# imalexlee/simple-vk-renderer

Hardware: AMD Instinct MI355X
Metric: shaded fragments/s (higher is better)
Workload: dtype f32

## Files before the change

simple-vk-renderer_amd/csrc/k_bin.hip:

```cpp
#include <hip/hip_ext.h>

#include <algorithm>

#include "svr_bin.h"
#include "svr_clip.h"
#include "svr_launch.h"

namespace svr {

__device__ __forceinline__ EdgeSet load_edges(const TriRec* rec) {
  EdgeSet e;
  const double2* p = reinterpret_cast<const double2*>(rec);
  double2 a = p[2], b = p[3], c = p[4], d = p[5];
  e.A0 = a.x; e.A1 = a.y; e.A2 = b.x; e.B0 = b.y; e.B1 = c.x; e.B2 = c.y; e.C0 = d.x; e.C1 = d.y;
  e.C2 = rec->C[2];
  return e;
}

struct RecBox {
  int minx, miny, maxx, maxy;
  uint32_t flags;
  bool valid;
};
__device__ __forceinline__ RecBox load_box(const TriRec* rec) {
  uint4 h = *reinterpret_cast<const uint4*>(rec);
  RecBox b;
  b.minx = (int)(int16_t)(h.x & 0xffffu);
  b.miny = (int)(int16_t)(h.x >> 16);
  b.maxx = (int)(int16_t)(h.y & 0xffffu);
  b.maxy = (int)(int16_t)(h.y >> 16);
  b.flags = h.w;
  b.valid = b.minx <= b.maxx;
  return b;
}

__device__ __forceinline__ void bin_one(const FrameParams& P, uint32_t r, int minx, int miny, int maxx, int maxy, uint32_t binbase,
                                        const EdgeSet& e, uint32_t n_setup) {
  const uint32_t lane = threadIdx.x & 63u;
  const unsigned long long below = (1ull << lane) - 1ull;
// ... 89 lines not shown
      bool made = false;
      uint32_t rec = 0, transparent = 0;
      if (worker && i + 1 < np) {
        const DrawDesc& d = P.draws[draw];
        ScreenV s0 = to_screen(poly[0].clip, hw, hh), s1 = to_screen(poly[i].clip, hw, hh), s2 = to_screen(poly[i + 1].clip, hw, hh);
        if (s0.ok && s1.ok && s2.ok && poly[0].clip[3] > 0.0f && poly[i].clip[3] > 0.0f && poly[i + 1].clip[3] > 0.0f) {
          rec = P.n_tris + first + used;
          uint4* dst = reinterpret_cast<uint4*>(P.recs + rec);
          if (setup_triangle(P, &poly[0], &poly[i], &poly[i + 1], s0, s1, s2, make_key(seq, d.flags, P.tex[d.tex], true), d.flags, P.tex[d.tex],
                             *reinterpret_cast<uint4(*)[16]>(dst), &L.geom[lane])) {
            made = true;
            used++;
            if (IDS) *reinterpret_cast<uint2*>(dst + REC_ID_PIECE) = make_uint2(d.pad, prim);
            transparent = MV ? bin_base<true>(P, d.flags) : ((d.flags & F_TRANSPARENT) ? 1u : 0u);
            if (P.instrument) atomicAdd(&P.counters->binned, 1ull);
          }
        }
      }
      __builtin_amdgcn_fence(__ATOMIC_RELEASE, "wavefront");
      __builtin_amdgcn_wave_barrier();
      for (unsigned long long todo = __ballot(made); todo; todo &= todo - 1ull) {
        const int l = __ffsll((long long)todo) - 1;
        const TriGeom& gm = L.geom[l];
        EdgeSet e;
        e.A0 = gm.A[0]; e.A1 = gm.A[1]; e.A2 = gm.A[2]; e.B0 = gm.B[0]; e.B1 = gm.B[1]; e.B2 = gm.B[2];
        e.C0 = gm.C[0]; e.C1 = gm.C[1]; e.C2 = gm.C[2];
        bin_one(P, (uint32_t)__shfl((int)rec, l), gm.minx, gm.miny, gm.maxx, gm.maxy, MV ? (uint32_t)__shfl((int)transparent, l) : (__shfl((int)transparent, l) ? P.n_tiles : 0u), e, n_setup);
      }
      __builtin_amdgcn_wave_barrier();
    }
    if (worker && np >= 3) {
      for (uint32_t k = used; k < want; k++) store_invalid(P.recs + P.n_tris + first + k);
      uint4 link;
      link.x = 1u;
      link.y = 0u;
      link.z = P.n_tris + first;
      link.w = used;
      *reinterpret_cast<uint4*>(P.recs + seq) = link;
    }
  }
}

template <bool IDS, bool MV>
__device__ __forceinline__ void count_main(const FrameParams& P, uint32_t big_blocks, uint32_t clip_blocks) {
  __shared__ ClipLds s_clip;
  if (P.counters->overflow) return;
  if (blockIdx.x < big_blocks) {
    bin_big<MV>(P, (blockIdx.x * blockDim.x + threadIdx.x) >> 6, (big_blocks * blockDim.x) >> 6);
    return;
// ... 183 lines not shown
```

simple-vk-renderer_amd/csrc/k_geometry.hip:

```cpp
#include <algorithm>

#include "svr_bin.h"
#include "svr_clip.h"
#include "svr_launch.h"

namespace svr {

__device__ __forceinline__ bool chunk_can_be_seen(const FrameParams& P, const float* mvp, const float lo[3], const float hi[3], uint32_t lane) {
  const float px = (lane & 4u) ? hi[0] : lo[0], py = (lane & 2u) ? hi[1] : lo[1], pz = (lane & 1u) ? hi[2] : lo[2];
  float c[4];
  matvec4(mvp, px, py, pz, 1.0f, c);
  const float inv_hw = 2.0f / (float)P.W, inv_hh = 2.0f / (float)P.H;
  const float x_lo = ((float)P.sx - 1.0f) * inv_hw - 1.0f, x_hi = ((float)(P.sx + P.sw) + 1.0f) * inv_hw - 1.0f;
  const float y_lo = ((float)P.sy - 1.0f) * inv_hh - 1.0f, y_hi = ((float)(P.sy + P.sh) + 1.0f) * inv_hh - 1.0f;
  const unsigned long long corners = 0xffull;
  const bool out_near = c[2] > c[3], out_far = c[2] < 0.0f;
  const bool out_l = c[0] < x_lo * c[3], out_r = c[0] > x_hi * c[3];
  const bool out_t = c[1] < y_lo * c[3], out_b = c[1] > y_hi * c[3];
  const bool gone = (__ballot(out_near) & corners) == corners || (__ballot(out_far) & corners) == corners ||
                    (__ballot(out_l) & corners) == corners || (__ballot(out_r) & corners) == corners ||
                    (__ballot(out_t) & corners) == corners || (__ballot(out_b) & corners) == corners;
  if (gone) return false;
  if (P.rstride > 1u) {
    const bool front = (__ballot(c[3] > 0.0f) & corners) == corners;
// ... 191 lines not shown
      piece[REC_ID_PIECE].x = d.pad;
      piece[REC_ID_PIECE].y = tri;
    }
    if (ok && P.instrument) atomicAdd(&P.counters->binned, 1ull);
    if (to_clip) {
      uint32_t slot = atomicAdd(&P.counters->n_clip, 1u);
      if (slot < P.clip_cap) {
        ClipItem it;
        it.draw = ch.draw;
        it.tri = tri;
        P.clip_queue[slot] = it;
      } else {
        atomicOr(&P.counters->overflow, 1u);
      }
    }
  }
  {
    const unsigned long long act = __ballot(tri < d.tri_count), okm = __ballot(ok);
    uint4* wave_recs = reinterpret_cast<uint4*>(P.recs + (d.tri_base + ch.first_tri));
    uint4* sl = s_tr[threadIdx.x >> 6];
    __builtin_amdgcn_fence(__ATOMIC_RELEASE, "workgroup");
    __builtin_amdgcn_wave_barrier();
#pragma unroll
    for (int half = 0; half < 2; half++) {
      if (DO && !IDS && half == 1) continue;
#pragma unroll
      for (uint32_t r = 0; r < 2u; r++) {
        __builtin_amdgcn_wave_barrier();
        if ((lane >> 5) == r) {
#pragma unroll
          for (int i = 0; i < 8; i++) sl[(lane & 31u) * 8u + ((uint32_t)i ^ (lane & 7u))] = piece[half * 8 + i];
        }
        __builtin_amdgcn_wave_barrier();
#pragma unroll
        for (int k = 0; k < 4; k++) {
          const uint32_t tl = (uint32_t)k * 8u + (lane >> 3), i = lane & 7u, t = 32u * r + tl;
          uint4 v = sl[tl * 8u + (i ^ (tl & 7u))];
          bool header = half == 0 && i == 0u;
          if (DO && (half == 0 ? i == 7u : i != REC_ID_PIECE - 8u)) continue;
          if ((act >> t) & 1ull)
            if (header || ((okm >> t) & 1ull)) wave_recs[t * 16u + (uint32_t)half * 8u + i] = v;
        }
      }
    }
  }
  TileRange tr = tile_range(P, g.minx, g.miny, g.maxx, g.maxy, ok);
  {
    bool big = ok && tr.nt > SMALL_MAX_TILES;
    unsigned long long m = __ballot(big);
    if (m) {
      uint32_t base = 0;
      if (lane == 0) base = atomicAdd(&P.counters->n_big, (uint32_t)__popcll(m));
      base = __shfl(base, 0);
      if (big) P.big_queue[base + (uint32_t)__popcll(m & ((1ull << lane) - 1ull))] = seq;
    }
  }
  EdgeSet e;
  e.A0 = g.A[0]; e.A1 = g.A[1]; e.A2 = g.A[2]; e.B0 = g.B[0]; e.B1 = g.B[1]; e.B2 = g.B[2];
  e.C0 = g.C[0]; e.C1 = g.C[1]; e.C2 = g.C[2];
  emit_small_pairs(P, ok && tr.nt <= SMALL_MAX_TILES, tr, g.minx, g.miny, g.maxx, g.maxy,
                   bin_base<MV>(P, d.flags), e, seq, s_tot);
}

__global__ __launch_bounds__(256) void mesh_vert_kernel(const SvrVertex* vtx, uint32_t first, uint32_t n,
                                                        const float* world16, const float* viewproj16,
                                                        const float* cf4, float* out_clip, float* out_var) {
  uint32_t i = blockIdx.x * blockDim.x + threadIdx.x;
  if (i >= n) return;
  float world[16], viewproj[16], mvp[16], cf[4];
  for (int k = 0; k < 16; k++) {
    world[k] = world16[k];
    viewproj[k] = viewproj16[k];
  }
  for (int k = 0; k < 4; k++) cf[k] = cf4[k];
  matmul4(viewproj, world, mvp);
  VertexRaw v = load_vertex(vtx, first + i);
  VOut o;
  mesh_vert(v, mvp, world, cf, o);
  reinterpret_cast<float4*>(out_clip)[i] = make_float4(o.clip[0], o.clip[1], o.clip[2], o.clip[3]);
  reinterpret_cast<float4*>(out_var)[2 * i] = make_float4(o.attr[0], o.attr[1], o.attr[2], o.attr[3]);
  reinterpret_cast<float4*>(out_var)[2 * i + 1] = make_float4(o.attr[4], o.attr[5], o.attr[6], o.attr[7]);
}
// ... 85 lines not shown
```

simple-vk-renderer_amd/csrc/k_tile.hip:

```cpp
#include <hip/hip_ext.h>

#include <cstdlib>
#include <type_traits>

#include "svr_launch.h"
#include "svr_pixel.h"
#include "svr_span.h"

namespace svr {

constexpr uint32_t REC_COMMON = 0x80000000u;
#ifndef SVR_PRIO_COST
#define SVR_PRIO_COST 200u
#endif
constexpr int BATCH = 64;
constexpr uint32_t SREC = 7;

constexpr float kG0 = 0x1.c51282p-2f, kG1 = -0x1.14a3a2p-2f, kG2 = 0x1.37536ap-3f, kG3 = -0x1.778474p-5f;

__device__ __forceinline__ float lod_from_rho2(float rho2) {
  uint32_t bits = f2u(rho2);
  int e = (int)(bits >> 23) - 127;
  float m = u2f((bits & 0x7fffffu) | 0x3f800000u);
  float t = m - 1.0f;
  float g = fmaf(fmaf(fmaf(kG3, t, kG2), t, kG1), t, kG0);
  float s = t * (1.0f - t);
  float l = fmaf(s, g, t);
  float lam = 0.5f * ((float)e + l);
  lam = (rho2 <= 0x1p+100f) ? lam : 50.0f;
  lam = (rho2 >= 0x1p-100f) ? lam : -50.0f;
  return lam;
}

__device__ __forceinline__ float lerpf(float a, float b, float t) { return fmaf(t, b - a, a); }
__device__ __forceinline__ float clamp_med3(float x, float lo, float hi) { return __builtin_amdgcn_fmed3f(x, lo, hi); }
__device__ __forceinline__ double top_left_bias(uint32_t flags, uint32_t bit) { return (double)((flags / bit) & 1u); }

struct TexD {
  uint32_t base_off;
  uint32_t w, h, lw, lh, levels, filters;
  float min_lod, max_lod;
};

struct Taps {
  uint32_t o00, o10, o01, o11;
  float alpha, beta;
};
__device__ __forceinline__ Taps level_taps(int wl, int hl, uint32_t plw, uint32_t base, bool linear, float u, float v) {
  float U = (u - floorf(u)) * (float)wl;
  float V = (v - floorf(v)) * (float)hl;
  float Uh = U - 0.5f, Vh = V - 0.5f;
  float fu = floorf(linear ? Uh : U), fv = floorf(linear ? Vh : V);
  Taps tp;
  tp.alpha = linear ? Uh - fu : 0.0f;
  tp.beta = linear ? Vh - fv : 0.0f;
  int i0 = (int)fu, j0 = (int)fv;
  int i1 = linear ? i0 + 1 : i0, j1 = linear ? j0 + 1 : j0;
  if (i0 < 0) i0 += wl;
  if (i0 >= wl) i0 -= wl;
// ... 59 lines not shown
    tx.y = lerpf(tx.y, bilerp(l00, l10, l01, l11, 1, tl.alpha, tl.beta), delta);
    tx.z = lerpf(tx.z, bilerp(l00, l10, l01, l11, 2, tl.alpha, tl.beta), delta);
  }
  return tx;
}

__device__ __forceinline__ float interp3(float a0, float da1, float da2, float b1, float b2, float r) {
  return fmaf(b2, da2, fmaf(b1, da1, a0)) * r;
}

struct FragAttr {
  float b1, b2, r, u, v, nx, ny, nz, light, cr, cg, cb, won;
};

__device__ __forceinline__ float quad_partner_x(float v) { return u2f((uint32_t)__builtin_amdgcn_mov_dpp((int)f2u(v), 0xB1, 0xf, 0xf, true)); }
__device__ __forceinline__ float quad_partner_y(float v) { return u2f((uint32_t)__builtin_amdgcn_mov_dpp((int)f2u(v), 0x128, 0xf, 0xf, true)); }
template <bool TRACE, bool COMMON = false, bool ATTR = false>
__device__ __forceinline__ float4 shade_pixel(const FrameParams& P, uint32_t rec, int px, int py, float* trace, const bool quads = false,
                                              FragAttr* fa = nullptr) {
  const TriRec* tr = P.recs + rec;
  const uint4* q4 = reinterpret_cast<const uint4*>(tr);
  const float4* f4 = reinterpret_cast<const float4*>(tr);
  const double2* d2 = reinterpret_cast<const double2*>(tr);
  uint4 hdr = q4[0];
  float4 zrow = f4[1];
  double2 c2 = d2[2], c3 = d2[3], c4 = d2[4], c5 = d2[5], c6 = d2[6];
  uint4 td = q4[7];
  float4 s0 = f4[8], s1 = f4[9], s2 = f4[10], s3 = f4[11], s4 = f4[12], s5 = f4[13], s6 = f4[14];
  uint32_t flags = hdr.w;
  float inv_area = zrow.w;
  double A1, B1, A2, B2, e1, e2;
  double C1 = c5.y, C2 = c6.x;
  A1 = c2.y; B1 = c4.x; A2 = c3.x; B2 = c4.y;
  double dx = (double)px, dy = (double)py;
  e1 = fma(A1, dx, fma(B1, dy, C1)) + top_left_bias(flags, F_T1);
  e2 = fma(A2, dx, fma(B2, dy, C2)) + top_left_bias(flags, F_T2);
  TexD t;
  t.base_off = (uint32_t)(unsigned long long)__double_as_longlong(c6.y);
  const uint32_t tk = (uint32_t)((unsigned long long)__double_as_longlong(c6.y) >> 32);
  t.w = td.x & 0xffffu;
  t.h = td.x >> 16;
  t.lw = td.y & 0xffu;
  t.lh = (td.y >> 8) & 0xffu;
  t.levels = (td.y >> 16) & 0xffu;
  t.filters = td.y >> 24;
  t.min_lod = u2f(td.z);
  t.max_lod = u2f(td.w);
  float b1 = (float)e1 * inv_area, b2 = (float)e2 * inv_area;
  float q0 = s0.x, dq1 = s0.y, dq2 = s0.z;
  const float qq = fmaf(b2, dq2, fmaf(b1, dq1, q0));
  float hb1 = 0.0f, hb2 = 0.0f, vb1 = 0.0f, vb2 = 0.0f, hq = 1.0f, vq = 1.0f, hr = 0.0f, vr = 0.0f;
  auto partners = [&]() {
    if (COMMON) {
      const int sx = (int)((uint32_t)px << 31), sy = (int)((uint32_t)py << 31);
      auto flip = [](double a, int s) { return __hiloint2double(__double2hiint(a) ^ s, __double2loint(a)); };
      hb1 = (float)(e1 + flip(A1, sx)) * inv_area, hb2 = (float)(e2 + flip(A2, sx)) * inv_area;
      vb1 = (float)(e1 + flip(B1, sy)) * inv_area, vb2 = (float)(e2 + flip(B2, sy)) * inv_area;
    } else {
      double sxp = (px & 1) ? -1.0 : 1.0, syp = (py & 1) ? -1.0 : 1.0;
// ... 17 lines not shown
    vr = rcp_ieee(vq);
  }
  float uh, vh, uv_, vv_;
  if (quads) {
    uh = quad_partner_x(u), vh = quad_partner_x(v);
    uv_ = quad_partner_y(u), vv_ = quad_partner_y(v);
  } else {
    if (COMMON) {
      partners();
      hr = rcp_in_window(hq);
      vr = rcp_in_window(vq);
    }
    uh = interp3(s2.y, s4.y, s6.y, hb1, hb2, hr), vh = interp3(s2.z, s4.z, s6.z, hb1, hb2, hr);
    uv_ = interp3(s2.y, s4.y, s6.y, vb1, vb2, vr), vv_ = interp3(s2.z, s4.z, s6.z, vb1, vb2, vr);
  }
  float dudx = (COMMON || !(px & 1)) ? (uh - u) : (u - uh);
  float dvdx = (COMMON || !(px & 1)) ? (vh - v) : (v - vh);
  float dudy = (COMMON || !(py & 1)) ? (uv_ - u) : (u - uv_);
  float dvdy = (COMMON || !(py & 1)) ? (vv_ - v) : (v - vv_);
  float W0 = (float)t.w, H0 = (float)t.h;
  float mx = COMMON ? ldexpf(dudx, (int)t.lw) : dudx * W0, my = COMMON ? ldexpf(dvdx, (int)t.lh) : dvdx * H0;
  float nx_ = COMMON ? ldexpf(dudy, (int)t.lw) : dudy * W0, ny_ = COMMON ? ldexpf(dvdy, (int)t.lh) : dvdy * H0;
  float rho2 = fmaxf(fmaf(mx, mx, my * my), fmaf(nx_, nx_, ny_ * ny_));
  float lambda = COMMON ? clamp_med3(lod_from_rho2(rho2), t.min_lod, t.max_lod) : fminf(fmaxf(lod_from_rho2(rho2), t.min_lod), t.max_lod);
  const bool linear = COMMON ? true : (((lambda <= 0.0f) ? (t.filters & 1u) : ((t.filters >> 1) & 1u)) != 0u);
  int q = COMMON ? (int)(tk >> 24) : (int)t.levels - 1;
  const bool mip_linear = COMMON ? true : (((t.filters >> 2) & 1u) != 0u);
  int dn = min(max((int)ceilf(lambda + 0.5f) - 1, 0), q);
  float lc = COMMON ? clamp_med3(lambda, 0.0f, (float)q) : fminf(fmaxf(lambda, 0.0f), (float)q);
  float fl = floorf(lc);
  int dhi = mip_linear ? (int)fl : dn;
  float delta = mip_linear ? lc - fl : 0.0f;
  int dlo = mip_linear ? min(dhi + 1, q) : dn;
  float us = (COMMON || fabsf(u) < 8388608.0f) ? u : 0.0f, vs = (COMMON || fabsf(v) < 8388608.0f) ? v : 0.0f;
  float4 tx;
  if constexpr (COMMON) {
    tx = common_texture(P.tex_arena, t.base_off, tk, td.y, dhi, dlo, delta, us, vs);
  } else {
    const int whi = (int)max(t.w >> dhi, 1u), hhi = (int)max(t.h >> dhi, 1u);
    const uint32_t bhi = t.base_off + mip_offset(t.lw, t.lh, (uint32_t)dhi);
    const uint32_t plw_hi = level_lw(t.lw, (uint32_t)dhi);
    Taps th = level_taps(whi, hhi, plw_hi, bhi, linear, us, vs);
    const uint8_t* tb = P.tex_arena;
    uint32_t h00 = texel(tb, th.o00), h10 = texel(tb, th.o10), h01 = texel(tb, th.o01), h11 = texel(tb, th.o11);
    const bool two_levels = __any(delta != 0.0f);
    Taps tl = th;
    uint32_t l00 = 0, l10 = 0, l01 = 0, l11 = 0;
// ... 98 lines not shown
    bool hidden = false;
    uint32_t gone = 0;
    uint32_t zb = 0, claim = 0;
    if (lane < cnt) {
      uint4 h = s_cov[lane * SREC];
      int minx = (int)(int16_t)(h.x & 0xffffu), miny = (int)(int16_t)(h.x >> 16);
      int maxx = (int)(int16_t)(h.y & 0xffffu), maxy = (int)(int16_t)(h.y >> 16);
      cx0 = max(minx, tx0);
      const int cx1 = min(maxx, tx0 + TILE - 1);
      const int cy0 = max(miny, ry0), cy1 = min(maxy, ry0 + nrows - 1);
      cw = (cx1 >= cx0 && cy1 >= cy0) ? cx1 - cx0 + 1 : 0;
      if (HIZ && cw) {
        const float4 zr = reinterpret_cast<const float4*>(s_cov)[lane * SREC + 1u];
        const float eps = (fabsf(zr.x) + fabsf(zr.y) + fabsf(zr.z)) * 0x1p-21f;
        zb = f2u(fmaxf(fmaxf(zr.x, fmaxf(zr.x + zr.y, zr.x + zr.z)) + eps, 0.0f));
        if (minx <= tx0 && maxx >= tx0 + TILE - 1 && miny <= ry0 && maxy >= ry0 + nrows - 1) {
          const double* dd = reinterpret_cast<const double*>(s_cov + lane * SREC);
          const float x0 = (float)tx0, x1 = (float)(tx0 + TILE - 1), y0 = (float)ry0, y1 = (float)(ry0 + nrows - 1);
          bool all_in = true;
          float slack = 0.0f;
          float bc[2][4];
#pragma unroll
          for (int i = 0; i < 3; i++) {
            const float A = (float)dd[4 + i], B = (float)dd[7 + i], C = (float)dd[10 + i] + ((i == 1 && (h.w & F_T1)) || (i == 2 && (h.w & F_T2)) ? 1.0f : 0.0f);
            const float M = (fabsf(C) + fmaxf(fabsf(A * x0), fabsf(A * x1)) + fmaxf(fabsf(B * y0), fabsf(B * y1))) * 0x1p-21f;
            const float e00 = fmaf(A, x0, fmaf(B, y0, C)), e10 = fmaf(A, x1, fmaf(B, y0, C));
            const float e01 = fmaf(A, x0, fmaf(B, y1, C)), e11 = fmaf(A, x1, fmaf(B, y1, C));
            all_in = all_in && fminf(fminf(e00, e10), fminf(e01, e11)) >= M + 1.0f;
            if (i) {
              bc[i - 1][0] = e00 * zr.w; bc[i - 1][1] = e10 * zr.w; bc[i - 1][2] = e01 * zr.w; bc[i - 1][3] = e11 * zr.w;
              slack = fmaxf(slack, M * zr.w);
            }
          }
          if (all_in) {
            float zmin = fmaf(bc[1][0], zr.z, fmaf(bc[0][0], zr.y, zr.x));
            zmin = fminf(zmin, fmaf(bc[1][1], zr.z, fmaf(bc[0][1], zr.y, zr.x)));
            zmin = fminf(zmin, fmaf(bc[1][2], zr.z, fmaf(bc[0][2], zr.y, zr.x)));
            zmin = fminf(zmin, fmaf(bc[1][3], zr.z, fmaf(bc[0][3], zr.y, zr.x)));
            zmin -= eps + 2.0f * slack * (fabsf(zr.y) + fabsf(zr.z));
            claim = f2u(fminf(fmaxf(zmin, 0.0f), 1.0f));
          }
        }
      }
    }
    if (HIZ) {
      unsigned long long claims = __ballot(claim != 0u);
      while (claims) {
// ... 48 lines not shown
      uint32_t item = c * 64u + lane;
      uint32_t j = item >> sh, band = item & ((1u << sh) - 1u);
      bool act = item < items;
      uint32_t pos = 0;
#pragma unroll
      for (uint32_t step = 32; step >= 1; step >>= 1) {
        uint32_t v = __shfl(inc, (int)min(pos + step - 1u, 63u));
        if (pos + step <= 64u && v <= j) pos += step;
      }
      uint32_t i = min(pos, 63u);
      uint32_t excl = __shfl(inc, (int)i) - (uint32_t)__shfl(cw, (int)i);
      int col = __shfl(cx0, (int)i) + (int)(j - excl);
      if (!act) continue;
      const uint4* rec = s_cov + i * SREC;
      uint4 h = rec[0];
      int miny = (int)(int16_t)(h.x >> 16), maxy = (int)(int16_t)(h.y >> 16);
      int y0 = max(miny, ry0 + (int)band * band_rows), y1 = min(maxy, ry0 + (int)band * band_rows + band_rows - 1);
      if (y0 > y1) continue;
      uint32_t key = h.z, flags = h.w;
      float4 zr = reinterpret_cast<const float4*>(rec)[1];
      const double2* d = reinterpret_cast<const double2*>(rec);
      double2 c2 = d[2], c3 = d[3], c4 = d[4], c5 = d[5], c6 = d[6];
      double B0 = c3.y, B1 = c4.x, B2 = c4.y;
      double u1 = top_left_bias(flags, F_T1), u2 = top_left_bias(flags, F_T2);
      double dx = (double)col, dy = (double)y0;
      double f0 = fma(c2.x, dx, fma(B0, dy, c5.x));
      double f1 = fma(c2.y, dx, fma(B1, dy, c5.y));
      double f2 = fma(c3.x, dx, fma(B2, dy, c6.x));
      int k0, kn;
      svr_span::column_span(f0, f1, f2, B0, B1, B2, y1 - y0 + 1, k0, kn);
      if (kn == 0) continue;
      if (INSTR) n_raster += (uint32_t)kn;
      const double dk = (double)k0;
      double g1 = fma(B1, dk, f1) + u1, g2 = fma(B2, dk, f2) + u2;
      unsigned long long* cell = s_depth + (y0 + k0 - ty0) * TILE + (col - tx0);
      for (; kn > 0; kn--) {
        float b1 = (float)g1 * zr.w, b2 = (float)g2 * zr.w;
        float z = fmaf(b2, zr.z, fmaf(b1, zr.y, zr.x));
        z = fminf(fmaxf(z, 0.0f), 1.0f) + 0.0f;
        if (INSTR && (flags >> 31) && f2u(z) >= (uint32_t)(*cell >> 32)) n_hiz_bad++;
        atomicMax(cell, ((unsigned long long)f2u(z) << 32) | key);
        g1 += B1;
        g2 += B2;
        cell += TILE;
      }
    }
  }
}

__device__ __forceinline__ uint32_t resolve_record(const FrameParams& P, uint32_t rec, int px, int py) {
  uint4 h = *reinterpret_cast<const uint4*>(P.recs + rec);
  if ((int)(int16_t)(h.x & 0xffffu) <= (int)(int16_t)(h.y & 0xffffu)) return rec;
  double dx = (double)px, dy = (double)py;
  for (uint32_t c = 0; c < h.w; c++) {
    const TriRec* t = P.recs + h.z + c;
    if (t->minx > t->maxx || px < t->minx || px > t->maxx || py < t->miny || py > t->maxy) continue;
    if (fma(t->A[0], dx, fma(t->B[0], dy, t->C[0])) >= 0.0 && fma(t->A[1], dx, fma(t->B[1], dy, t->C[1])) >= 0.0 &&
        fma(t->A[2], dx, fma(t->B[2], dy, t->C[2])) >= 0.0)
      return h.z + c;
  }
  return rec;
}

constexpr uint32_t SORT_CAP = SPLIT_SORT_MAX;
constexpr uint32_t RANK_SORT_MAX = 1024;
#ifndef SVR_HIZ_FILTER_MIN
#define SVR_HIZ_FILTER_MIN 1024
#endif
constexpr uint32_t HIZ_AVG_ENTRIES = 96;
constexpr uint32_t HIZ_FILTER_MIN = SVR_HIZ_FILTER_MIN;
constexpr uint32_t QUARTER_LIST_CAP = 3808;
constexpr uint32_t QUEUE_CAP = 128;

template <int FMT, bool INSTR>
__device__ __forceinline__ void flush_fragments(const FrameParams& P, typename Codec<FMT>::enc_t* col, uint2* q,
                                                float4* s_src, uint32_t& qn, int tx0, int by0,
                                                uint32_t lane, uint32_t& n_shaded) {
  typedef Codec<FMT> CD;
  uint32_t cnt = min(qn, 64u);
  bool act = lane < cnt;
  uint2 e = q[act ? lane : 0u];
// ... 112 lines not shown
      while (c * 64u < total) {
        uint32_t j = c * 64u + lane;
        bool act = j < total;
        uint32_t pos = 0;
#pragma unroll
        for (uint32_t step = 32; step >= 1; step >>= 1) {
          uint32_t v = __shfl(inc, (int)min(pos + step - 1u, 63u));
          if (pos + step <= 64u && v <= j) pos += step;
        }
        uint32_t i = min(pos, 63u);
        uint32_t excl = __shfl(inc, (int)i) - (uint32_t)__shfl(cw, (int)i);
        int colx = __shfl(cx0, (int)i) + (int)(j - excl) - tx0;
        colx = act ? colx : 0;
        const uint4* rec = s_cov + i * SREC;
        uint4 h = rec[0];
        int y0 = (int)(int16_t)(h.x >> 16), y1 = (int)(int16_t)(h.y >> 16);
        uint32_t flags = h.w, ri = s_idx[i];
        float4 zr = reinterpret_cast<const float4*>(rec)[1];
        const double2* d = reinterpret_cast<const double2*>(rec);
        double2 c2 = d[2], c3 = d[3], c4 = d[4], c5 = d[5], c6 = d[6];
        double B0 = c3.y, B1 = c4.x, B2 = c4.y;
        double dx = (double)(tx0 + colx), dy = (double)(by0 + t);
        double f0 = fma(c2.x, dx, fma(B0, dy, c5.x));
        const double u1 = top_left_bias(flags, F_T1), u2 = top_left_bias(flags, F_T2);
        double g1 = fma(c2.y, dx, fma(B1, dy, c5.y));
        double g2 = fma(c3.x, dx, fma(B2, dy, c6.x));
#pragma unroll 1
        for (; t < rpw; t++) {
          int y = by0 + t;
          bool inside = act && y >= y0 && y <= y1 && f0 >= 0.0 && g1 >= 0.0 && g2 >= 0.0;
          if (INSTR) n_raster += inside ? 1u : 0u;
          float b1 = (float)(g1 + u1) * zr.w, b2 = (float)(g2 + u2) * zr.w;
          float z = fmaf(b2, zr.z, fmaf(b1, zr.y, zr.x));
          z = fminf(fmaxf(z, 0.0f), 1.0f) + 0.0f;
          bool pass = inside && f2u(z) >= s_z[(y - ty0) * TILE + colx];
          unsigned long long m = __ballot(pass);
          f0 += B0;
          g1 += B1;
          g2 += B2;
          if (m) {
            if (pass) q[qn + (uint32_t)__popcll(m & below)] = make_uint2((uint32_t)(t * TILE + colx), ri | ((h.z & 2u) ? REC_COMMON : 0u));
            qn += (uint32_t)__popcll(m);
            if (qn >= 64u) {
              full = true;
              t++;
              break;
            }
          }
        }
        if (full) break;
        t = 0;
        c++;
      }
      if (!full) break;
      flush_fragments<FMT, INSTR>(P, col, q, s_src, qn, tx0, by0, lane, n_shaded);
// ... 954 lines not shown
```

simple-vk-renderer_amd/csrc/svr_api.hip:

```cpp
#include <algorithm>
#include <chrono>
#include <cmath>
#include <cstdio>
#include <numeric>

#include "svr_context.h"
#include "svr_cull.h"

using namespace svr;

namespace {
thread_local std::string g_err;
}
int svr::fail(int code, const std::string& msg) {
  g_err = msg;
  return code;
}
int svr::hip_fail(hipError_t e, const char* what) {
  return fail(e == hipErrorOutOfMemory ? SVR_ERR_OUT_OF_MEMORY : SVR_ERR_DEVICE, std::string(what) + ": " + hipGetErrorString(e));
}

namespace {

uint16_t host_f32_to_f16(float f) {
// ... 12 lines not shown
  int shift = 126 - (int)(ax >> 23);
  uint32_t h = mant >> shift, rem = mant & ((1u << shift) - 1u), half = 1u << (shift - 1);
  if (rem > half || (rem == half && (h & 1u))) h++;
  return (uint16_t)(sign | h);
}

MeshRes* get_mesh(SvrContext* ctx, SvrMesh h) {
  if (h == 0 || h > ctx->meshes.size() || !ctx->meshes[h - 1].alive) return nullptr;
  return &ctx->meshes[h - 1];
}
ImageRes* get_image(SvrContext* ctx, SvrImage h) {
  if (h == 0 || h > ctx->images.size() || !ctx->images[h - 1].alive) return nullptr;
  return &ctx->images[h - 1];
}

TexBinding make_binding(const ImageRes& im, const SvrSamplerDesc& s) {
  TexBinding tb;
  std::memset(&tb, 0, sizeof(tb));
  uint32_t filters = (uint32_t)s.mag_filter | ((uint32_t)s.min_filter << 1) | ((uint32_t)s.mipmap_mode << 2);
  tb.base_off = im.arena_off;
  tb.pad0 = tex_consts(im.lw, im.lh, im.levels);
  tb.wh = im.w | (im.h << 16);
  tb.info = im.lw | (im.lh << 8) | (im.levels << 16) | (filters << 24);
  tb.min_lod = binding_min_lod(s.min_lod, s.max_lod);
  tb.max_lod = s.max_lod;
  return tb;
}

constexpr size_t ARENA_MAX = (size_t)0xffffff00u;
constexpr size_t ARENA_ALIGN = 256;

int arena_alloc(SvrContext* ctx, size_t bytes, uint32_t* off) {
  bytes = (bytes + ARENA_ALIGN - 1) & ~(ARENA_ALIGN - 1);
  for (size_t i = 0; i < ctx->tex_holes.size(); i++) {
    auto& h = ctx->tex_holes[i];
    if (h.second >= bytes) {
      *off = (uint32_t)h.first;
      h.first += bytes;
      h.second -= bytes;
      if (h.second == 0) ctx->tex_holes.erase(ctx->tex_holes.begin() + (long)i);
      return SVR_OK;
    }
  }
  if (ctx->tex_arena_top + bytes > ARENA_MAX)
    return fail(SVR_ERR_OUT_OF_MEMORY, "svr_create_image: more than 4 GiB of texels in one context");
  if (ctx->tex_arena_top + bytes > ctx->tex_arena_cap) {
    size_t want = std::max(ctx->tex_arena_cap * 2, ctx->tex_arena_top + bytes);
    want = std::min(ARENA_MAX, (want + ((size_t)64 << 20) - 1) & ~(((size_t)64 << 20) - 1));
// ... 1435 lines not shown
```

simple-vk-renderer_amd/csrc/svr_bin.h:

```cpp
#pragma once
#include "svr_device.h"

namespace svr {

constexpr int SMALL_MAX_TILES = 16;

struct EdgeSet {
  double A0, A1, A2, B0, B1, B2, C0, C1, C2;
};

__device__ __forceinline__ bool box_overlaps(const EdgeSet& e, int x0, int y0, int x1, int y1) {
  double fx0 = (double)x0, fx1 = (double)x1, fy0 = (double)y0, fy1 = (double)y1;
  double m0 = fma(e.A0, e.A0 >= 0.0 ? fx1 : fx0, fma(e.B0, e.B0 >= 0.0 ? fy1 : fy0, e.C0));
  double m1 = fma(e.A1, e.A1 >= 0.0 ? fx1 : fx0, fma(e.B1, e.B1 >= 0.0 ? fy1 : fy0, e.C1));
  double m2 = fma(e.A2, e.A2 >= 0.0 ? fx1 : fx0, fma(e.B2, e.B2 >= 0.0 ? fy1 : fy0, e.C2));
  return m0 >= 0.0 && m1 >= 0.0 && m2 >= 0.0;
}

struct TileRange {
  int tx0, ty0, ntx, nt;
};
__device__ __forceinline__ TileRange tile_range(const FrameParams& P, int minx, int miny, int maxx, int maxy, bool valid) {
  TileRange t;
  t.tx0 = (minx - (int)P.sx) >> TILE_SHIFT;
  int l1;
  local_tile_rows(P, miny, maxy, t.ty0, l1);
  t.ntx = ((maxx - (int)P.sx) >> TILE_SHIFT) - t.tx0 + 1;
  int nty = l1 - t.ty0 + 1;
  t.nt = (valid && nty > 0) ? t.ntx * nty : 0;
  return t;
}

// ... 59 lines not shown
```

simple-vk-renderer_amd/csrc/svr_device.h:

```cpp
#pragma once

#include <hip/hip_runtime.h>
#include <stdint.h>

#include "../../include/svr.h"

namespace svr {

constexpr int TILE = 32;
constexpr int TILE_SHIFT = 5;
constexpr int WAVE = 64;
constexpr float GUARD = 16384.0f;
constexpr uint32_t NO_REC = 0xffffffffu;
#ifndef SVR_RCP_VARIANT
#define SVR_RCP_VARIANT 1
#endif

enum PipelineKind : uint32_t { PIPE_MESH = 0, PIPE_COLORED_TRIANGLE = 1, PIPE_TEX_IMAGE = 2 };

constexpr uint32_t F_T1 = 1u;
constexpr uint32_t F_T2 = 2u;
constexpr uint32_t F_KIND_SHIFT = 4;
constexpr uint32_t F_TRANSPARENT = 256u;
constexpr uint32_t F_VIEW_SHIFT = 24;
// ... 91 lines not shown
}
__host__ __device__ inline uint32_t packed_level_lw(uint32_t info, uint32_t level) {
  const int d = (int)(info & 0xffu) - (int)level;
  return (uint32_t)(d > (int)TEX_TILE_LW ? d : (int)TEX_TILE_LW);
}
__host__ __device__ inline uint32_t packed_level_lh(uint32_t info, uint32_t level) {
  const int d = (int)((info >> 8) & 0xffu) - (int)level;
  return (uint32_t)(d > (int)TEX_TILE_LH ? d : (int)TEX_TILE_LH);
}
__host__ __device__ inline uint32_t packed_level_bytes(uint32_t k, uint32_t level) {
  const uint32_t a = k & 0xffu, b = (k >> 8) & 0xffu, cc = (k >> 16) & 0xffu;
  return 4u << (cc - (level < a ? level : a) - (level < b ? level : b));
}
__host__ __device__ inline uint32_t packed_mip_offset(uint32_t k, uint32_t level) {
  const uint32_t a = k & 0xffu, b = (k >> 8) & 0xffu, cc = (k >> 16) & 0xffu;
  const uint32_t l1 = level < a ? level : a, l2 = level < b ? level : b;
  uint32_t off = (0x2aaaaaaau >> (31u - 2u * l1)) << ((cc + 4u - 2u * l1) & 31u);
  if (level > a) off += (8u << (cc - 2u * a)) - (8u << (cc - a - l2));
  if (level > b) off += (level - b) * TEX_TILE_BYTES;
  return off;
}

__host__ __device__ inline float binding_min_lod(float lo, float hi) { return lo <= hi ? lo : hi; }

__host__ __device__ inline bool frag_ranges_ok(float q0, float dq1, float dq2, double A1, double B1, double A2, double B2, float inv_area,
                                               const float (&uv)[6]) {
  const float fa1 = (float)A1, fb1 = (float)B1, fa2 = (float)A2, fb2 = (float)B2;
  const float gx = (fa1 * dq1 + fa2 * dq2) * inv_area, gy = (fb1 * dq1 + fb2 * dq2) * inv_area;
  const float a1 = fa1 < 0.0f ? -fa1 : fa1, b1 = fb1 < 0.0f ? -fb1 : fb1, a2 = fa2 < 0.0f ? -fa2 : fa2, b2 = fb2 < 0.0f ? -fb2 : fb2;
  const float steps = ((a1 > b1 ? a1 : b1) * (dq1 < 0.0f ? -dq1 : dq1) + (a2 > b2 ? a2 : b2) * (dq2 < 0.0f ? -dq2 : dq2)) * inv_area;
  const float q1 = q0 + dq1, q2 = q0 + dq2;
  const float lo0 = q0 < q1 ? (q0 < q2 ? q0 : q2) : (q1 < q2 ? q1 : q2), hi0 = q0 > q1 ? (q0 > q2 ? q0 : q2) : (q1 > q2 ? q1 : q2);
  const float ax = gx < 0.0f ? -gx : gx, ay = gy < 0.0f ? -gy : gy, G = ax > ay ? ax : ay;
  const float mag = steps + (q0 < 0.0f ? -q0 : q0) + (dq1 < 0.0f ? -dq1 : dq1) + (dq2 < 0.0f ? -dq2 : dq2);
  const float allow = mag * 0x1p-19f + 0x1p-100f;
  const float lo = lo0 - G - allow, hi = hi0 + G + allow;
  float sum = 0.0f;
  for (int i = 0; i < 6; i++) sum += uv[i] < 0.0f ? -uv[i] : uv[i];
  return lo >= 0x1p-94f && hi <= 0x1p95f && mag <= 0x1p100f && sum * (lo + 0x1p-18f * hi) < 4194304.0f * lo;
}

struct TriRec {
  int16_t minx, miny, maxx, maxy;
  uint32_t key;
  uint32_t flags;
  float z0, dz1, dz2, inv_area;
  double A[3], B[3], C[3];
  uint32_t tex_off, tex_pad;
  uint32_t tex_wh, tex_info;
  float tex_min_lod, tex_max_lod;
  float q0, dq1, dq2;
  float a0[8], da1[8], da2[8];
  float pad2;
  uint32_t object, primitive;
  float pad3[2];
};
static_assert(sizeof(TriRec) == 256, "TriRec layout");
static_assert(offsetof(TriRec, object) == 240, "TriRec layout: the ID words are piece 15's x and y");
constexpr uint32_t REC_ID_PIECE = offsetof(TriRec, object) / 16u;
static_assert(offsetof(TriRec, A) == 32 && offsetof(TriRec, tex_off) == 104 && offsetof(TriRec, tex_wh) == 112 &&
                  offsetof(TriRec, q0) == 128, "TriRec layout");

struct ClipItem {
  uint32_t draw;
  uint32_t tri;
};

struct Counters {
  uint32_t n_clip;
  uint32_t n_extra;
  uint32_t total_entries;
  uint32_t overflow;
  unsigned long long rasterized;
  unsigned long long shaded;
  unsigned long long binned;
  uint32_t n_big;
  uint32_t n_pairs;
  uint32_t n_pairs_rest;
  uint32_t sort_used;
  uint32_t n_split;
  uint32_t cost_sum;
  uint32_t flat_draws;
  uint32_t flat_tris;
  uint32_t flat_chunks;
// ... 102 lines not shown
  return (int)P.sy + (ty * (int)P.rstride + (int)P.roff) * TILE;
}
__device__ __forceinline__ void local_tile_rows(const FrameParams& P, int miny, int maxy, int& l0, int& l1) {
  const int g0 = (miny - (int)P.sy) >> TILE_SHIFT, g1 = (maxy - (int)P.sy) >> TILE_SHIFT;
  l0 = g0;
  l1 = g1;
  if (P.rstride > 1u) {
    const int s = (int)P.rstride, b = g1 - (int)P.roff;
    l0 = (g0 - (int)P.roff + s - 1) / s;
    l1 = b < 0 ? -1 : b / s;
  }
}

template <bool MV>
__device__ __forceinline__ uint32_t bin_base(const FrameParams& P, uint32_t flags) {
  uint32_t b = (flags & F_TRANSPARENT) ? P.n_tiles : 0u;
  if (MV) b += (flags >> F_VIEW_SHIFT) * P.layer_rows * P.tiles_x;
  return b;
}

__device__ __forceinline__ float u2f(uint32_t u) { return __uint_as_float(u); }
__device__ __forceinline__ uint32_t f2u(float f) { return __float_as_uint(f); }

template <int VARIANT>
__device__ __forceinline__ float rcp_refined(float x) {
  float y = __builtin_amdgcn_rcpf(x);
  float r = fmaf(-x, y, 1.0f);
  y = fmaf(r, y, y);
  if (VARIANT == 2) {
    r = fmaf(-x, y, 1.0f);
    y = fmaf(r, y, y);
  }
  return y;
}
__device__ __forceinline__ bool rcp_fast_ok(float x) {
  return ((f2u(x) >> 23) & 0xffu) - 32u <= 190u;
}
__device__ __forceinline__ float rcp_ieee(float x) {
#ifdef SVR_AB_PLAIN_DIV
  return 1.0f / x;
#endif
  if (__builtin_expect(!rcp_fast_ok(x), 0)) return 1.0f / x;
  return rcp_refined<SVR_RCP_VARIANT>(x);
}
__device__ __forceinline__ float rcp_in_window(float x) {
#ifdef SVR_AB_PLAIN_DIV
// ... 155 lines not shown
  pminx = max(pminx, (int)P.sx);
  pminy = max(pminy, (int)P.sy);
  pmaxx = min(pmaxx, (int)(P.sx + P.sw) - 1);
  pmaxy = min(pmaxy, (int)(P.sy + P.sh) - 1);
  if (pminx > pmaxx || pminy > pmaxy) return false;
  if (P.rstride > 1u) {
    int l0, l1;
    local_tile_rows(P, pminy, pmaxy, l0, l1);
    if (l0 > l1) return false;
  }

  int Xs[3] = {X0, X1, X2}, Ys[3] = {Y0, Y1, Y2};
  double A[3], B[3], C[3];
  uint32_t flags = draw_flags;
#pragma unroll
  for (int i = 0; i < 3; i++) {
    int a = (i + 1) % 3, b = (i + 2) % 3;
    long long dx = (long long)Xs[b] - Xs[a], dy = (long long)Ys[b] - Ys[a];
    long long Ae = -dy, Be = dx, Ce = -dx * Ys[a] + dy * Xs[a];
    bool top_left = (dy < 0) || (dy == 0 && dx > 0);
    long long Cu = Ce + 128 * (Ae + Be);
    A[i] = (double)(Ae * 256);
    B[i] = (double)(Be * 256);
    C[i] = (double)(Cu + (top_left ? 0 : -1));
    if (!top_left && i == 1) flags |= F_T1;
    if (!top_left && i == 2) flags |= F_T2;
  }
  float inv_area = rcp_ieee((float)(double)area2);
  if (geom) {
    geom->minx = pminx; geom->miny = pminy; geom->maxx = pmaxx; geom->maxy = pmaxy;
#pragma unroll
    for (int i = 0; i < 3; i++) {
      geom->A[i] = A[i]; geom->B[i] = B[i]; geom->C[i] = C[i];
    }
  }

  const float rw0 = s0.rw;
  if (key & 2u) {
    const float uv[6] = {v0->attr[6], v0->attr[7], v1->attr[6], v1->attr[7], v2->attr[6], v2->attr[7]};
    if (!frag_ranges_ok(rw0, rw1 - rw0, rw2 - rw0, A[1], B[1], A[2], B[2], inv_area, uv)) key &= ~2u;
  }

  uint4 h;
  h.x = ((uint32_t)(uint16_t)pminx) | ((uint32_t)(uint16_t)pminy << 16);
  h.y = ((uint32_t)(uint16_t)pmaxx) | ((uint32_t)(uint16_t)pmaxy << 16);
  h.z = key;
  h.w = flags;
// ... 4 lines not shown
    return make_uint4((uint32_t)ua, (uint32_t)(ua >> 32), (uint32_t)ub, (uint32_t)(ub >> 32));
  };
  rec[2] = pack2(A[0], A[1]);
  rec[3] = pack2(A[2], B[0]);
  rec[4] = pack2(B[1], B[2]);
  rec[5] = pack2(C[0], C[1]);
  {
    unsigned long long uc = (unsigned long long)__double_as_longlong(C[2]);
    rec[6] = make_uint4((uint32_t)uc, (uint32_t)(uc >> 32), tex.base_off, tex.pad0);
  }
  rec[7] = make_uint4(tex.wh, tex.info, f2u(tex.min_lod), f2u(tex.max_lod));
  float sh[32];
  sh[0] = rw0;
  sh[1] = rw1 - rw0;
  sh[2] = rw2 - rw0;
#pragma unroll
  for (int k = 0; k < 8; k++) {
    const float a1 = flip ? v2->attr[k] : v1->attr[k], a2 = flip ? v1->attr[k] : v2->attr[k];
    float p0 = v0->attr[k] * rw0, p1 = a1 * rw1, p2 = a2 * rw2;
    sh[3 + k] = p0;
    sh[11 + k] = p1 - p0;
    sh[19 + k] = p2 - p0;
  }
#pragma unroll
  for (int k = 27; k < 32; k++) sh[k] = 0.0f;
#pragma unroll
  for (int k = 0; k < 8; k++) rec[8 + k] = make_uint4(f2u(sh[4 * k]), f2u(sh[4 * k + 1]), f2u(sh[4 * k + 2]), f2u(sh[4 * k + 3]));
  return true;
}

}
```

Before: 49.44 billion.

## Fold top-left bias out of stored edge constants and trim shading header loads

```diff
diff --git a/simple-vk-renderer_amd/csrc/k_bin.hip b/simple-vk-renderer_amd/csrc/k_bin.hip
--- a/simple-vk-renderer_amd/csrc/k_bin.hip
+++ b/simple-vk-renderer_amd/csrc/k_bin.hip
@@ -9,12 +9,10 @@
 namespace svr {
 
 __device__ __forceinline__ EdgeSet load_edges(const TriRec* rec) {
-  EdgeSet e;
   const double2* p = reinterpret_cast<const double2*>(rec);
   double2 a = p[2], b = p[3], c = p[4], d = p[5];
-  e.A0 = a.x; e.A1 = a.y; e.A2 = b.x; e.B0 = b.y; e.B1 = c.x; e.B2 = c.y; e.C0 = d.x; e.C1 = d.y;
-  e.C2 = rec->C[2];
-  return e;
+  const double A[3] = {a.x, a.y, b.x}, B[3] = {b.y, c.x, c.y}, C[3] = {d.x, d.y, rec->C[2]};
+  return edge_set(A, B, C);
 }
 
 struct RecBox {
@@ -150,9 +148,7 @@
       for (unsigned long long todo = __ballot(made); todo; todo &= todo - 1ull) {
         const int l = __ffsll((long long)todo) - 1;
         const TriGeom& gm = L.geom[l];
-        EdgeSet e;
-        e.A0 = gm.A[0]; e.A1 = gm.A[1]; e.A2 = gm.A[2]; e.B0 = gm.B[0]; e.B1 = gm.B[1]; e.B2 = gm.B[2];
-        e.C0 = gm.C[0]; e.C1 = gm.C[1]; e.C2 = gm.C[2];
+        const EdgeSet e = edge_set(gm);
         bin_one(P, (uint32_t)__shfl((int)rec, l), gm.minx, gm.miny, gm.maxx, gm.maxy, MV ? (uint32_t)__shfl((int)transparent, l) : (__shfl((int)transparent, l) ? P.n_tiles : 0u), e, n_setup);
       }
       __builtin_amdgcn_wave_barrier();
diff --git a/simple-vk-renderer_amd/csrc/k_geometry.hip b/simple-vk-renderer_amd/csrc/k_geometry.hip
--- a/simple-vk-renderer_amd/csrc/k_geometry.hip
+++ b/simple-vk-renderer_amd/csrc/k_geometry.hip
@@ -237,7 +237,7 @@
     __builtin_amdgcn_fence(__ATOMIC_RELEASE, "workgroup");
     __builtin_amdgcn_wave_barrier();
 #pragma unroll
-    for (int half = 0; half < 2; half++) {
+    for (int half = 1; half >= 0; half--) {
       if (DO && !IDS && half == 1) continue;
 #pragma unroll
       for (uint32_t r = 0; r < 2u; r++) {
@@ -270,9 +270,7 @@
       if (big) P.big_queue[base + (uint32_t)__popcll(m & ((1ull << lane) - 1ull))] = seq;
     }
   }
-  EdgeSet e;
-  e.A0 = g.A[0]; e.A1 = g.A[1]; e.A2 = g.A[2]; e.B0 = g.B[0]; e.B1 = g.B[1]; e.B2 = g.B[2];
-  e.C0 = g.C[0]; e.C1 = g.C[1]; e.C2 = g.C[2];
+  const EdgeSet e = edge_set(g);
   emit_small_pairs(P, ok && tr.nt <= SMALL_MAX_TILES, tr, g.minx, g.miny, g.maxx, g.maxy,
                    bin_base<MV>(P, d.flags), e, seq, s_tot);
 }
diff --git a/simple-vk-renderer_amd/csrc/k_tile.hip b/simple-vk-renderer_amd/csrc/k_tile.hip
--- a/simple-vk-renderer_amd/csrc/k_tile.hip
+++ b/simple-vk-renderer_amd/csrc/k_tile.hip
@@ -16,25 +16,8 @@
 constexpr int BATCH = 64;
 constexpr uint32_t SREC = 7;
 
-constexpr float kG0 = 0x1.c51282p-2f, kG1 = -0x1.14a3a2p-2f, kG2 = 0x1.37536ap-3f, kG3 = -0x1.778474p-5f;
-
-__device__ __forceinline__ float lod_from_rho2(float rho2) {
-  uint32_t bits = f2u(rho2);
-  int e = (int)(bits >> 23) - 127;
-  float m = u2f((bits & 0x7fffffu) | 0x3f800000u);
-  float t = m - 1.0f;
-  float g = fmaf(fmaf(fmaf(kG3, t, kG2), t, kG1), t, kG0);
-  float s = t * (1.0f - t);
-  float l = fmaf(s, g, t);
-  float lam = 0.5f * ((float)e + l);
-  lam = (rho2 <= 0x1p+100f) ? lam : 50.0f;
-  lam = (rho2 >= 0x1p-100f) ? lam : -50.0f;
-  return lam;
-}
-
 __device__ __forceinline__ float lerpf(float a, float b, float t) { return fmaf(t, b - a, a); }
 __device__ __forceinline__ float clamp_med3(float x, float lo, float hi) { return __builtin_amdgcn_fmed3f(x, lo, hi); }
-__device__ __forceinline__ double top_left_bias(uint32_t flags, uint32_t bit) { return (double)((flags / bit) & 1u); }
 
 struct TexD {
   uint32_t base_off;
@@ -140,19 +123,23 @@
   const uint4* q4 = reinterpret_cast<const uint4*>(tr);
   const float4* f4 = reinterpret_cast<const float4*>(tr);
   const double2* d2 = reinterpret_cast<const double2*>(tr);
-  uint4 hdr = q4[0];
-  float4 zrow = f4[1];
+  uint4 hdr = make_uint4(0u, 0u, 0u, 0u);
+  float4 zrow = make_float4(0.f, 0.f, 0.f, 0.f);
+  if (!COMMON) {
+    hdr = q4[0];
+    zrow = f4[1];
+  }
   double2 c2 = d2[2], c3 = d2[3], c4 = d2[4], c5 = d2[5], c6 = d2[6];
   uint4 td = q4[7];
   float4 s0 = f4[8], s1 = f4[9], s2 = f4[10], s3 = f4[11], s4 = f4[12], s5 = f4[13], s6 = f4[14];
   uint32_t flags = hdr.w;
-  float inv_area = zrow.w;
+  float inv_area = COMMON ? s6.w : zrow.w;
   double A1, B1, A2, B2, e1, e2;
   double C1 = c5.y, C2 = c6.x;
   A1 = c2.y; B1 = c4.x; A2 = c3.x; B2 = c4.y;
   double dx = (double)px, dy = (double)py;
-  e1 = fma(A1, dx, fma(B1, dy, C1)) + top_left_bias(flags, F_T1);
-  e2 = fma(A2, dx, fma(B2, dy, C2)) + top_left_bias(flags, F_T2);
+  e1 = fma(A1, dx, fma(B1, dy, C1));
+  e2 = fma(A2, dx, fma(B2, dy, C2));
   TexD t;
   t.base_off = (uint32_t)(unsigned long long)__double_as_longlong(c6.y);
   const uint32_t tk = (uint32_t)((unsigned long long)__double_as_longlong(c6.y) >> 32);
@@ -216,7 +203,7 @@
   float mx = COMMON ? ldexpf(dudx, (int)t.lw) : dudx * W0, my = COMMON ? ldexpf(dvdx, (int)t.lh) : dvdx * H0;
   float nx_ = COMMON ? ldexpf(dudy, (int)t.lw) : dudy * W0, ny_ = COMMON ? ldexpf(dvdy, (int)t.lh) : dvdy * H0;
   float rho2 = fmaxf(fmaf(mx, mx, my * my), fmaf(nx_, nx_, ny_ * ny_));
-  float lambda = COMMON ? clamp_med3(lod_from_rho2(rho2), t.min_lod, t.max_lod) : fminf(fmaxf(lod_from_rho2(rho2), t.min_lod), t.max_lod);
+  float lambda = COMMON ? clamp_med3(lod_from_rho2<false>(rho2), t.min_lod, t.max_lod) : fminf(fmaxf(lod_from_rho2(rho2), t.min_lod), t.max_lod);
   const bool linear = COMMON ? true : (((lambda <= 0.0f) ? (t.filters & 1u) : ((t.filters >> 1) & 1u)) != 0u);
   int q = COMMON ? (int)(tk >> 24) : (int)t.levels - 1;
   const bool mip_linear = COMMON ? true : (((t.filters >> 2) & 1u) != 0u);
@@ -361,7 +348,7 @@
           float bc[2][4];
 #pragma unroll
           for (int i = 0; i < 3; i++) {
-            const float A = (float)dd[4 + i], B = (float)dd[7 + i], C = (float)dd[10 + i] + ((i == 1 && (h.w & F_T1)) || (i == 2 && (h.w & F_T2)) ? 1.0f : 0.0f);
+            const float A = (float)dd[4 + i], B = (float)dd[7 + i], C = (float)dd[10 + i];
             const float M = (fabsf(C) + fmaxf(fabsf(A * x0), fabsf(A * x1)) + fmaxf(fabsf(B * y0), fabsf(B * y1))) * 0x1p-21f;
             const float e00 = fmaf(A, x0, fmaf(B, y0, C)), e10 = fmaf(A, x1, fmaf(B, y0, C));
             const float e01 = fmaf(A, x0, fmaf(B, y1, C)), e11 = fmaf(A, x1, fmaf(B, y1, C));
@@ -456,17 +443,17 @@
       const double2* d = reinterpret_cast<const double2*>(rec);
       double2 c2 = d[2], c3 = d[3], c4 = d[4], c5 = d[5], c6 = d[6];
       double B0 = c3.y, B1 = c4.x, B2 = c4.y;
-      double u1 = top_left_bias(flags, F_T1), u2 = top_left_bias(flags, F_T2);
       double dx = (double)col, dy = (double)y0;
       double f0 = fma(c2.x, dx, fma(B0, dy, c5.x));
-      double f1 = fma(c2.y, dx, fma(B1, dy, c5.y));
-      double f2 = fma(c3.x, dx, fma(B2, dy, c6.x));
+      double h1 = fma(c2.y, dx, fma(B1, dy, c5.y));
+      double h2 = fma(c3.x, dx, fma(B2, dy, c6.x));
+      double f1 = h1 - edge_bias(flags, F_T1), f2 = h2 - edge_bias(flags, F_T2);
       int k0, kn;
       svr_span::column_span(f0, f1, f2, B0, B1, B2, y1 - y0 + 1, k0, kn);
       if (kn == 0) continue;
       if (INSTR) n_raster += (uint32_t)kn;
       const double dk = (double)k0;
-      double g1 = fma(B1, dk, f1) + u1, g2 = fma(B2, dk, f2) + u2;
+      double g1 = fma(B1, dk, h1), g2 = fma(B2, dk, h2);
       unsigned long long* cell = s_depth + (y0 + k0 - ty0) * TILE + (col - tx0);
       for (; kn > 0; kn--) {
         float b1 = (float)g1 * zr.w, b2 = (float)g2 * zr.w;
@@ -489,8 +476,9 @@
   for (uint32_t c = 0; c < h.w; c++) {
     const TriRec* t = P.recs + h.z + c;
     if (t->minx > t->maxx || px < t->minx || px > t->maxx || py < t->miny || py > t->maxy) continue;
-    if (fma(t->A[0], dx, fma(t->B[0], dy, t->C[0])) >= 0.0 && fma(t->A[1], dx, fma(t->B[1], dy, t->C[1])) >= 0.0 &&
-        fma(t->A[2], dx, fma(t->B[2], dy, t->C[2])) >= 0.0)
+    const uint32_t fl = t->flags;
+    if (fma(t->A[0], dx, fma(t->B[0], dy, t->C[0])) >= 0.0 && fma(t->A[1], dx, fma(t->B[1], dy, t->C[1])) >= edge_bias(fl, F_T1) &&
+        fma(t->A[2], dx, fma(t->B[2], dy, t->C[2])) >= edge_bias(fl, F_T2))
       return h.z + c;
   }
   return rec;
@@ -649,15 +637,15 @@
         double B0 = c3.y, B1 = c4.x, B2 = c4.y;
         double dx = (double)(tx0 + colx), dy = (double)(by0 + t);
         double f0 = fma(c2.x, dx, fma(B0, dy, c5.x));
-        const double u1 = top_left_bias(flags, F_T1), u2 = top_left_bias(flags, F_T2);
+        const double u1 = edge_bias(flags, F_T1), u2 = edge_bias(flags, F_T2);
         double g1 = fma(c2.y, dx, fma(B1, dy, c5.y));
         double g2 = fma(c3.x, dx, fma(B2, dy, c6.x));
 #pragma unroll 1
         for (; t < rpw; t++) {
           int y = by0 + t;
-          bool inside = act && y >= y0 && y <= y1 && f0 >= 0.0 && g1 >= 0.0 && g2 >= 0.0;
+          bool inside = act && y >= y0 && y <= y1 && f0 >= 0.0 && g1 >= u1 && g2 >= u2;
           if (INSTR) n_raster += inside ? 1u : 0u;
-          float b1 = (float)(g1 + u1) * zr.w, b2 = (float)(g2 + u2) * zr.w;
+          float b1 = (float)g1 * zr.w, b2 = (float)g2 * zr.w;
           float z = fmaf(b2, zr.z, fmaf(b1, zr.y, zr.x));
           z = fminf(fmaxf(z, 0.0f), 1.0f) + 0.0f;
           bool pass = inside && f2u(z) >= s_z[(y - ty0) * TILE + colx];
diff --git a/simple-vk-renderer_amd/csrc/svr_api.hip b/simple-vk-renderer_amd/csrc/svr_api.hip
--- a/simple-vk-renderer_amd/csrc/svr_api.hip
+++ b/simple-vk-renderer_amd/csrc/svr_api.hip
@@ -58,8 +58,7 @@
   tb.pad0 = tex_consts(im.lw, im.lh, im.levels);
   tb.wh = im.w | (im.h << 16);
   tb.info = im.lw | (im.lh << 8) | (im.levels << 16) | (filters << 24);
-  tb.min_lod = binding_min_lod(s.min_lod, s.max_lod);
-  tb.max_lod = s.max_lod;
+  if (!binding_lod_range(binding_min_lod(s.min_lod, s.max_lod), s.max_lod, tb.min_lod, tb.max_lod)) tb.info |= TEX_WIDE_LODS << 24;
   return tb;
 }
 
diff --git a/simple-vk-renderer_amd/csrc/svr_bin.h b/simple-vk-renderer_amd/csrc/svr_bin.h
--- a/simple-vk-renderer_amd/csrc/svr_bin.h
+++ b/simple-vk-renderer_amd/csrc/svr_bin.h
@@ -8,6 +8,15 @@
 struct EdgeSet {
   double A0, A1, A2, B0, B1, B2, C0, C1, C2;
 };
+__device__ __forceinline__ EdgeSet edge_set(const double (&A)[3], const double (&B)[3], const double (&C)[3]) {
+  EdgeSet e;
+  e.A0 = A[0]; e.A1 = A[1]; e.A2 = A[2]; e.B0 = B[0]; e.B1 = B[1]; e.B2 = B[2];
+  e.C0 = C[0];
+  e.C1 = C[1] - edge_bias(A[1], B[1]);
+  e.C2 = C[2] - edge_bias(A[2], B[2]);
+  return e;
+}
+__device__ __forceinline__ EdgeSet edge_set(const TriGeom& g) { return edge_set(g.A, g.B, g.C); }
 
 __device__ __forceinline__ bool box_overlaps(const EdgeSet& e, int x0, int y0, int x1, int y1) {
   double fx0 = (double)x0, fx1 = (double)x1, fy0 = (double)y0, fy1 = (double)y1;
diff --git a/simple-vk-renderer_amd/csrc/svr_device.h b/simple-vk-renderer_amd/csrc/svr_device.h
--- a/simple-vk-renderer_amd/csrc/svr_device.h
+++ b/simple-vk-renderer_amd/csrc/svr_device.h
@@ -137,6 +137,13 @@
 }
 
 __host__ __device__ inline float binding_min_lod(float lo, float hi) { return lo <= hi ? lo : hi; }
+constexpr float LOD_SELECT = 50.0f;
+constexpr uint32_t TEX_WIDE_LODS = 8u;
+__host__ __device__ inline bool binding_lod_range(float lo, float hi, float& out_lo, float& out_hi) {
+  out_lo = (hi >= -LOD_SELECT && lo < -LOD_SELECT) ? -LOD_SELECT : lo;
+  out_hi = (lo <= LOD_SELECT && hi > LOD_SELECT) ? LOD_SELECT : hi;
+  return out_lo >= -LOD_SELECT && out_hi <= LOD_SELECT;
+}
 
 __host__ __device__ inline bool frag_ranges_ok(float q0, float dq1, float dq2, double A1, double B1, double A2, double B2, float inv_area,
                                                const float (&uv)[6]) {
@@ -175,6 +182,9 @@
 constexpr uint32_t REC_ID_PIECE = offsetof(TriRec, object) / 16u;
 static_assert(offsetof(TriRec, A) == 32 && offsetof(TriRec, tex_off) == 104 && offsetof(TriRec, tex_wh) == 112 &&
                   offsetof(TriRec, q0) == 128, "TriRec layout");
+static_assert(offsetof(TriRec, pad2) == 236, "TriRec layout: inv_area's second copy is piece 14's w");
+__host__ __device__ inline double edge_bias(uint32_t flags, uint32_t bit) { return (double)((flags / bit) & 1u); }
+__host__ __device__ inline double edge_bias(double A, double B) { return (A > 0.0 || (A == 0.0 && B > 0.0)) ? 0.0 : 1.0; }
 
 struct ClipItem {
   uint32_t draw;
@@ -323,6 +333,22 @@
 __device__ __forceinline__ float u2f(uint32_t u) { return __uint_as_float(u); }
 __device__ __forceinline__ uint32_t f2u(float f) { return __float_as_uint(f); }
 
+constexpr float kG0 = 0x1.c51282p-2f, kG1 = -0x1.14a3a2p-2f, kG2 = 0x1.37536ap-3f, kG3 = -0x1.778474p-5f;
+template <bool SELECTS = true>
+__device__ __forceinline__ float lod_from_rho2(float rho2) {
+  uint32_t bits = f2u(rho2);
+  int e = (int)(bits >> 23) - 127;
+  float m = u2f((bits & 0x7fffffu) | 0x3f800000u);
+  float t = m - 1.0f;
+  float g = fmaf(fmaf(fmaf(kG3, t, kG2), t, kG1), t, kG0);
+  float s = t * (1.0f - t);
+  float l = fmaf(s, g, t);
+  float lam = 0.5f * ((float)e + l);
+  if (SELECTS) lam = (rho2 <= 0x1p+100f) ? lam : LOD_SELECT;
+  lam = (rho2 >= 0x1p-100f) ? lam : -LOD_SELECT;
+  return lam;
+}
+
 template <int VARIANT>
 __device__ __forceinline__ float rcp_refined(float x) {
   float y = __builtin_amdgcn_rcpf(x);
@@ -524,7 +550,7 @@
     long long Cu = Ce + 128 * (Ae + Be);
     A[i] = (double)(Ae * 256);
     B[i] = (double)(Be * 256);
-    C[i] = (double)(Cu + (top_left ? 0 : -1));
+    C[i] = (double)(i == 0 ? Cu + (top_left ? 0 : -1) : Cu);
     if (!top_left && i == 1) flags |= F_T1;
     if (!top_left && i == 2) flags |= F_T2;
   }
@@ -575,11 +601,11 @@
     sh[11 + k] = p1 - p0;
     sh[19 + k] = p2 - p0;
   }
-#pragma unroll
-  for (int k = 27; k < 32; k++) sh[k] = 0.0f;
-#pragma unroll
-  for (int k = 0; k < 8; k++) rec[8 + k] = make_uint4(f2u(sh[4 * k]), f2u(sh[4 * k + 1]), f2u(sh[4 * k + 2]), f2u(sh[4 * k + 3]));
-  return true;
-}
-
-}
+  sh[27] = inv_area;
+#pragma unroll
+  for (int k = 28; k < 32; k++) sh[k] = 0.0f;
+#pragma unroll
+  for (int k = 0; k < 8; k++) rec[8 + k] = make_uint4(f2u(sh[4 * k]), f2u(sh[4 * k + 1]), f2u(sh[4 * k + 2]), f2u(sh[4 * k + 3]));  return true;
+}
+
+}
```

Measured after the change: 50.91 billion, median of 6. 3.0% higher.
